# imulki/serenade

Measured on AMD Instinct MI355X. Metric: mel frames/sec converted (UNet ODE + vocoder), 80x1024, higher is better.
Workload: dtype f32

## Files before the change

### include/serenade_hip.h

```cpp
#ifndef SERENADE_HIP_H
#define SERENADE_HIP_H

#include <stdint.h>

#ifdef __cplusplus
extern "C" {
#endif

#define SRN_ABI_VERSION 4
#define SRN_MAX_TAPS 16

enum { SRN_ACT_NONE = 0, SRN_ACT_LEAKY = 1, SRN_ACT_SILU = 2, SRN_ACT_MISH = 3 };
enum { SRN_RES_NONE = 0, SRN_RES_ADD = 1, SRN_RES_AXPY = 2 };
enum {
  SRN_POST_NONE = 0,
  SRN_POST_DIV = 1,
  SRN_POST_TANH = 2,
  SRN_POST_RELU = 3,
  SRN_POST_LEAKY = 4,
  SRN_POST_GELU = 5
};
enum {
  SRN_PREC_FP32 = 0,
  SRN_PREC_BF16X3 = 1,
  SRN_PREC_BF16X6 = 2
};
enum {
  SRN_ROUTE_AUTO = 0,
  SRN_ROUTE_TILED = 1,
  SRN_ROUTE_HALO = 2,
  SRN_ROUTE_GENERIC = 3,
  SRN_ROUTE_STRIP = 4,
  SRN_ROUTE_FAST_FP32 = 5
};
enum {
  SRN_FAMILY_GENERIC = 0,
  SRN_FAMILY_F32 = 1,
  SRN_FAMILY_FAST = 2,
  SRN_FAMILY_HALO = 3,
  SRN_FAMILY_STRIP = 4
};

typedef struct SrnConvParams {
  int32_t n_batch;
  int32_t n_head;
  int32_t T_in, T_out;
  int32_t C_in;
  int32_t C_in0;
  int32_t C_w;
  int32_t N;
  int32_t N_out;
  int32_t n_taps;
  int32_t tap_off[SRN_MAX_TAPS];
  int32_t in_stride;
  int32_t pad_reflect;
  int32_t w_nmajor;
  int32_t pro_act;
  float pro_slope;
  float alpha;
  float beta;
  int32_t geglu;
  int32_t res_mode;
  int32_t post;
  float post_div;
  int32_t out_t_stride, out_t_off;
  int32_t tile;
  const float* in0; int64_t in0_bs, in0_hs; int32_t ld_in0;
  const float* in1; int64_t in1_bs; int32_t ld_in1;
  const float* w;   int64_t w_bs, w_hs; int32_t ldw;
  const float* bias;
  const int32_t* len_in;
  const int32_t* len_out;
  const float* res;  int64_t res_bs, res_hs; int32_t ld_res;
  const float* res2; int64_t res2_bs; int32_t ld_res2;
  float* out; int64_t out_bs, out_hs; int32_t ld_out;
  int32_t precision;
  int32_t route;
  void* ws; int64_t ws_bytes;
  const void* w_hi; const void* w_lo;
  float* gn_partials;
  float* out_tr; int64_t out_tr_bs; int32_t ld_out_tr; int32_t out_tr_col0;
} SrnConvParams;

int srn_abi_version(void);
const char* srn_last_error(void);

int srn_conv_gemm(const SrnConvParams* p, void* stream);
int64_t srn_conv_gemm_workspace_bytes(const SrnConvParams* p);
int srn_conv_gemm_route(const SrnConvParams* p, int32_t out[3]);

int srn_gn_mish_apply(const float* x, const float* gn_partials, const float* gamma, const float* beta,
                      const float* time_bias, int64_t time_bias_bs, const int32_t* lens, float* y, int B, int T,
                      int C, int groups, float eps, int valid_stats, void* stream);

int srn_resblock_tail(const float* c2, const float* gn_partials, const float* gamma, const float* beta,
                      const int32_t* lens, const float* r, const float* scale, const float* shift, int64_t ld_ss,
                      float* y, int B, int T, int C, int groups, float gn_eps, float ln_eps, int valid_stats,
                      void* stream);

int srn_resblock_tail_ln(const float* c2, const float* gn_partials, const float* gamma, const float* beta,
                         const int32_t* lens, const float* r, const float* scale, const float* shift, int64_t ld_ss,
                         float* y, int B, int T, int C, int groups, float gn_eps, float ln_eps, int valid_stats,
                         const float* ln2_gamma, const float* ln2_beta, float* y2, float ln2_eps, void* stream);

int srn_layernorm(const float* x, const float* gamma, const float* beta, float* y, int64_t rows, int C, float eps,
                  void* stream);

int srn_softmax_rows(float* s, const int32_t* lens, int Z, int n_head, int L, int ld, void* stream);

int srn_sinusoidal_emb(const float* t, float* out, int n, int dim, int ld, float scale, void* stream);

int srn_copy_channels(const float* src, int64_t src_bs, int ld_src, int sc0, float* dst, int64_t dst_bs, int ld_dst,
                      int dc0, int B, int T, int C, void* stream);

int srn_scatter_rows(const float* src, int64_t src_bs, int ld_src, float* dst, int64_t dst_bs, int ld_dst, int dc0,
                     const int32_t* row_off, const int32_t* n_rows, int B, int T, int C, void* stream);

int srn_transpose_ct(const float* src, float* dst, int B, int R, int Cc, int64_t src_bs, int ld_src, int64_t dst_bs,
                     int ld_dst, void* stream);
#define SRN_TR_LIST_MAX 40
typedef struct SrnTransposeList {
  int32_t n;
  int32_t pad_;
  const float* src[SRN_TR_LIST_MAX];
  float* dst[SRN_TR_LIST_MAX];
  int64_t src_bs[SRN_TR_LIST_MAX], dst_bs[SRN_TR_LIST_MAX];
  int32_t B[SRN_TR_LIST_MAX], R[SRN_TR_LIST_MAX], Cc[SRN_TR_LIST_MAX];
  int32_t ld_src[SRN_TR_LIST_MAX], ld_dst[SRN_TR_LIST_MAX];
  int32_t first_block[SRN_TR_LIST_MAX + 1];
} SrnTransposeList;
int srn_transpose_multi(const SrnTransposeList* list, void* stream);

int srn_renorm(const float* x, const float* trg_scale, const float* trg_mean, const float* voc_mean,
               const float* voc_scale, float* y, int64_t rows, int C, void* stream);

int srn_out_conv_tanh(const float* x, const float* w, const float* bias, float* y, int B, int T, int C, int k,
                      float slope, void* stream);

typedef struct SrnResUnitParams {
  int32_t n_batch, T, C;
  int32_t k, dilation;
  float slope;
  const float* x; int64_t x_bs;
  const float* w1; const float* b1; const float* w2; const float* b2;
  const void* w1_hi; const void* w2_hi;
  const float* res2; int64_t res2_bs;
  float post_div;
  float* out; int64_t out_bs;
  int32_t precision;
  int32_t route;
} SrnResUnitParams;
enum { SRN_RESUNIT_ROUTE_SHARED = 1 };

int srn_hifigan_resunit(const SrnResUnitParams* p, void* stream);

int srn_pd_gather(const float* x, const float* d, float* out, int B, int T, int C, float dilation, float slope,
                  void* stream);

int srn_gru_recur_last(const float* gi, const float* w_hh_t, const float* b_hh, float* h, int B, int T, int H,
                       void* stream);

int srn_style_token_attention_kv(const float* ref, const float* wq_t, const float* bq, const float* k, const float* v,
                                 const float* wo_t, const float* bo, float* out, int B, int Dq, int n_tok, int F,
                                 int n_head, void* stream);

int srn_pad_signal(const float* x, float* out, int B, int n, int pad, int ld, int mode, void* stream);
int srn_logmel(const float* spec, const float* mel_t, float* out, int64_t frames, int n_bins, int ld, int n_mels,
               float eps, int log_mode, void* stream);
int srn_loudness(const float* spec, const float* a_weight_db, uint32_t* gmax_ws, float* out, int B, int frames,
                 int n_bins, int ld, float amin, float top_db, float add_eps, void* stream);

int srn_rowln_fwd(const float* x, const float* m, int64_t m_bs, const float* a, int64_t a_bs, float* y, int B, int T,
                  int C, float eps, void* stream);
int srn_rowln_bwd(const float* x, const float* dy, const float* m, int64_t m_bs, float* dx, float* partial, int B, int T,
                  int C, float eps, void* stream);
int srn_rowln_chunks(int T);
int srn_gn_mish_bwd_partial(const float* h, const float* dy, const float* mean, const float* rstd, const float* gamma,
                            const float* beta, const int32_t* lens, float* partial, int B, int T, int C, int groups,
                            void* stream);
int srn_gn_mish_bwd_apply(const float* h, const float* dy, const float* mean, const float* rstd, const float* gamma,
                          const float* beta, const float* gsum, const int32_t* lens, float* dh, int B, int T, int C,
                          int groups, void* stream);
int srn_gn_chunks(int T);
int srn_gn_stats(const float* partials, float* mean, float* rstd, int B, int T, int C, int groups, float eps,
                 void* stream);
int srn_chunk_colsum(const float* partial, const float* gamma, float* col, float* gsum, int B, int n_chunk, int C,
                     int groups, void* stream);
int srn_colsum(const float* x, float* partial, float* out, int B, int64_t R, int N, int ld, void* stream);
int srn_colsum_chunks(int64_t R);
int srn_softmax_bwd(const float* p, float* dp, int64_t rows, int L, int ld, float scale, void* stream);
int srn_geglu_fwd(const float* hg, float* a, int64_t rows, int inner, void* stream);
int srn_geglu_bwd(const float* hg, const float* da, float* dhg, int64_t rows, int inner, void* stream);
int srn_adamw(float* p, const float* g, float* m, float* v, int64_t n, float lr, float beta1, float beta2, float eps,
              float weight_decay, int step, float grad_scale, void* stream);
int srn_adamw_dyn(float* p, const float* g, float* m, float* v, int64_t n, float beta1, float beta2, float eps,
                  float weight_decay, const float* dyn, void* stream);
int srn_sumsq(const float* g, int64_t n, double* partial, void* stream);
int srn_dot(const float* a, const float* b, int64_t n, double* partial, void* stream);
#define SRN_COPY_LIST_MAX 160
typedef struct SrnCopyList {
  int32_t n;
  int32_t pad_;
  const void* src[SRN_COPY_LIST_MAX];
  int64_t off[SRN_COPY_LIST_MAX];
  int64_t len[SRN_COPY_LIST_MAX];
} SrnCopyList;
int srn_multi_copy(const SrnCopyList* list, float* dst, void* stream);
int srn_sumsq_blocks(int64_t n);
int srn_weight_norm_fwd(const float* v, const float* g, float* w_packed, float* wd, float* inv_norm, int N, int C, int k,
                        void* stream);
int srn_weight_norm_bwd(const float* dw_packed, const float* v, const float* g, const float* inv_norm, float* dv,
                        float* dg, int N, int C, int k, void* stream);

typedef struct SrnWorldParams {
  int32_t n_batch, max_frames;
  int32_t fs, fft_size;
  const double* x; int64_t x_bs; const int32_t* x_len;
  const double* f0; const double* t; int64_t f_bs;
  const int32_t* n_frames;
  const double* twiddle;
  double q1, f0_floor;
  double threshold;
  double unvoiced_db;
  const double* band_window; int32_t band_window_len;
  int32_t n_bands;
  double* out0; int64_t out0_bs; int32_t ld_out0;
  double* out1; int64_t out1_bs; int32_t ld_out1;
} SrnWorldParams;
int srn_world_cheaptrick(const SrnWorldParams* p, void* stream);
int srn_world_d4c(const SrnWorldParams* p, void* stream);
int srn_world_project(const double* in, int64_t rows, int K, int ld_in, const double* mat_t, int n_out, int take_log,
                      double* out, int ld_out, void* stream);
int srn_world_pack_features(const double* a, int na, const double* b, int nb, const double* mean, const double* scale,
                            float* out, int64_t rows, int ld_out, void* stream);
int srn_wave_to_f64(const float* wave, double* out, int64_t n, int pcm16, void* stream);
int srn_f0_match_length(const double* in, int64_t in_bs, const int32_t* n_in, double* out, int64_t out_bs,
                        const int32_t* n_out, int n_batch, int max_out, void* stream);
int srn_cont_f0(const double* f0, int64_t bs, const int32_t* n_frames, double* cf0, float* uv, int32_t* ok,
                int n_batch, void* stream);
typedef struct SrnExcitationParams {
  int32_t n_batch, max_frames, fs, hop;
  const double* f0;
  const double* df_f0;
  int64_t f_bs;
  const int32_t* n_frames;
  double* phase_ws;
  const float* noise;
  float* sine;
  float sine_amp, noise_amp;
  int32_t n_df;
  float* dfs[4];
  int32_t df_upsample[4];
  double dense_factors[4];
} SrnExcitationParams;
int srn_sifigan_excitation(const SrnExcitationParams* p, void* stream);

typedef struct SrnTnGemmParams {
  int32_t n_batch, n_head;
  int32_t n_items, T_a, T_b;
  int32_t stride, n_shifts;
  int32_t shift[SRN_MAX_TAPS];
  int32_t M, N;
  const float* a; int64_t a_bs, a_hs, a_is; int32_t lda;
  const float* b; int64_t b_bs, b_hs, b_is; int32_t ldb;
  float* out; int64_t out_bs, out_hs; int32_t ldc;
  float alpha;
  float* ws; int64_t ws_bytes;
  int32_t n_inner;
  int64_t a_is2, b_is2;
  const int32_t* len_b;
  float* colsum;
  int32_t route;
} SrnTnGemmParams;
enum { SRN_TN_ROUTE_GENERAL = 1 };
int srn_tn_gemm(const SrnTnGemmParams* p, void* stream);
int64_t srn_tn_gemm_workspace_bytes(const SrnTnGemmParams* p);

int srn_bn_chunks(int64_t rows);
int srn_bn_relu_fwd(const float* x, const float* gamma, const float* beta, float* run_mean, float* run_var,
                    float* partial, float* stats, float* y, int64_t rows, int C, float eps, float momentum, void* stream);
int srn_bn_relu_bwd(const float* x, const float* y, const float* dy, const float* stats, const float* gamma,
                    float* partial, float* sums, float* dx, int64_t rows, int C, void* stream);
int srn_im2col_s2(const float* x, float* col, int B, int H, int W, int C, int ld, void* stream);
int srn_col2im_s2(const float* col, float* dx, int B, int H, int W, int C, int ld, void* stream);
int srn_gru_train_fwd(const float* gi, const float* w_hh_t, const float* b_hh, float* hs, float* gates, int B, int T,
                      int H, void* stream);
int srn_gru_train_bwd(const float* dh_last, const float* w_hh, const float* hs, const float* gates, float* dgi,
                      float* dgh, int B, int T, int H, void* stream);
int srn_token_attn_fwd(const float* q, const float* k, const float* v, float* p, float* ctx, int B, int n_tok, int F,
                       int n_head, void* stream);
int srn_token_attn_bwd(const float* dctx, const float* q, const float* k, const float* v, const float* p, float* dq,
                       float* dk_part, float* dv_part, int B, int n_tok, int F, int n_head, void* stream);

int srn_frame_stats_chunks(int T);
int srn_cvec_conv0(const float* wave, int64_t wave_bs, int n, const int32_t* lens, const float* w, float* out,
                   double* partials, int B, int T0, int C, int k, int stride, void* stream);
int srn_channel_norm_gelu(const float* x, const double* partials, int n_chunks, const int32_t* lens,
                          const float* gamma, const float* beta, float* stats, float* y, int B, int T, int C, float eps,
                          void* stream);
int srn_posconv_gelu_res(const float* x, const int32_t* lens, const float* w, const float* bias, float* y, int B,
                         int T, int C, int groups, int k, int pad, void* stream);

int srn_pad_ragged(const float* x, int64_t x_bs, const int32_t* lens, float* out, int B, int n, int pad, int ld,
                   void* stream);
int srn_mel_db(const float* spec, int ld_spec, int n_bins, const float* mel_t, const int32_t* lens, unsigned* gmax_ws,
               float* out, int ld_out, int B, int T, int n_mels, float amin, float top_db, void* stream);
int srn_trans_conv0(const float* x, int64_t x_bs, int ld_x, const int32_t* lens, const float* w, const float* bias,
                    float* out, int B, int T, int F, int C, int dilation, void* stream);
int srn_trans_pool(const float* in, const int32_t* lens, float* out, int B, int T, int F_in, int C, int C_valid,
                   int flatten, int ld_out, void* stream);
int srn_bilstm_slices(int H);
int srn_bilstm_recur(const float* g, int64_t g_bs, int ld_g, const int32_t* lens, const float* w_hh_t, float* out,
                     int64_t out_bs, int ld_out, int B, int T, int H, void* stream);

#define SRN_PYIN_MAX_FRAME 4096
#define SRN_PYIN_MAX_PERIODS 1024
#define SRN_PYIN_MAX_STATES 4096
#define SRN_PYIN_MAX_THRESHOLDS 1024
int srn_pyin_observe(const float* x, int64_t x_bs, const int32_t* lens, const int32_t* frames, const double* thresholds,
                     const double* beta_probs, const double* boltz_fact, const double* boltz_exp,
                     const double* no_trough, double* obs, double* voiced_prob, int B, int N, int T, int frame_length,
                     int win_length, int hop_length, int pad, int min_period, int max_period, int n_thresholds,
                     double sr, double fmin, double bins_per_octave, int n_bins, void* stream);
int srn_pyin_viterbi(const double* obs, const double* voiced_prob, const int32_t* frames, const double* log_band,
                     const double* log_p_init, const double* freqs, double log_tiny, double fill_na, int fill_unvoiced,
                     uint16_t* ptr_ws, int32_t* states, double* f0, uint8_t* voiced_flag, int B, int T, int n_bins,
                     int width, void* stream);

#define SRN_HARVEST_MAX_TAPS 1024
#define SRN_HARVEST_MAX_WINDOW 1536
#define SRN_HARVEST_MAX_CAND 256
#define SRN_HARVEST_MAX_RATIO 12
#define SRN_HARVEST_SMOOTH_PAD 300
int srn_harvest_decimate(const void* x, int x_is_f64, int64_t x_bs, const int32_t* lens, const double* coef, double* ws,
                         int64_t ws_stride, double* y, int64_t y_bs, int B, int N, int ratio, int lag, void* stream);
int srn_harvest_channels(const double* y, int64_t y_bs, const int32_t* ylens, const int32_t* frames, const double* taps,
                         const int32_t* tap_off, const int32_t* half_len, const double* boundary, int max_half_len,
                         double* events, int64_t ev_cap, double* raw, int B, int ch0, int n_launch, int n_ch, int F1,
                         int max_ylen, double fs, double f0_floor, double f0_ceil, void* stream);
int srn_harvest_candidates(const double* raw, const int32_t* frames, double* official, double* cand, int B, int n_ch,
                           int F1, int n_base, void* stream);
int srn_harvest_refine(const double* y, int64_t y_bs, const int32_t* ylens, const int32_t* frames, const double* cand,
                       double* refined, double* score, int B, int F1, int n_cand, double fs, double f0_floor,
                       double f0_ceil, void* stream);
int srn_harvest_contour(const double* refined, const double* score, const int32_t* frames, const int32_t* out_frames,
                        const double* smooth_coef, double* cand2, double* score2, double* fbuf, double* pool,
                        int64_t pool_stride, int32_t* sections, int sec_cap, int32_t* status, double* f0_out,
                        int64_t out_stride, int B, int F1, int n_cand, int F_out, int voice_range_minimum,
                        double frame_period, void* stream);

#ifdef __cplusplus
}
#endif
#endif
```

### serenade_amd/_lib.py

```python
import ctypes
import os
from ctypes import POINTER, c_char_p, c_double, c_float, c_int, c_int32, c_int64, c_void_p

_HERE = os.path.dirname(os.path.abspath(__file__))
LIB_PATH = os.environ.get("SERENADE_AMD_LIB") or os.path.join(_HERE, "libserenade_hip.so")

SRN_MAX_TAPS = 16
ACT_NONE, ACT_LEAKY, ACT_SILU, ACT_MISH = 0, 1, 2, 3
RES_NONE, RES_ADD, RES_AXPY = 0, 1, 2
POST_NONE, POST_DIV, POST_TANH, POST_RELU, POST_LEAKY, POST_GELU = 0, 1, 2, 3, 4, 5
PREC_FP32, PREC_BF16X3, PREC_BF16X6 = 0, 1, 2
ROUTE_AUTO, ROUTE_TILED, ROUTE_HALO, ROUTE_GENERIC, ROUTE_STRIP, ROUTE_FAST_FP32 = 0, 1, 2, 3, 4, 5
FAMILY_GENERIC, FAMILY_F32, FAMILY_FAST, FAMILY_HALO, FAMILY_STRIP = 0, 1, 2, 3, 4
RESUNIT_ROUTE_SHARED = 1
TN_ROUTE_GENERAL = 1


class SrnConvParams(ctypes.Structure):
    _fields_ = [
        ("n_batch", c_int32), ("n_head", c_int32), ("T_in", c_int32), ("T_out", c_int32),
        ("C_in", c_int32), ("C_in0", c_int32), ("C_w", c_int32), ("N", c_int32), ("N_out", c_int32),
        ("n_taps", c_int32), ("tap_off", c_int32 * SRN_MAX_TAPS), ("in_stride", c_int32),
        ("pad_reflect", c_int32), ("w_nmajor", c_int32), ("pro_act", c_int32), ("pro_slope", c_float),
        ("alpha", c_float), ("beta", c_float), ("geglu", c_int32), ("res_mode", c_int32), ("post", c_int32), ("post_div", c_float),
        ("out_t_stride", c_int32), ("out_t_off", c_int32), ("tile", c_int32),
        ("in0", c_void_p), ("in0_bs", c_int64), ("in0_hs", c_int64), ("ld_in0", c_int32),
        ("in1", c_void_p), ("in1_bs", c_int64), ("ld_in1", c_int32),
        ("w", c_void_p), ("w_bs", c_int64), ("w_hs", c_int64), ("ldw", c_int32),
        ("bias", c_void_p), ("len_in", c_void_p), ("len_out", c_void_p),
        ("res", c_void_p), ("res_bs", c_int64), ("res_hs", c_int64), ("ld_res", c_int32),
        ("res2", c_void_p), ("res2_bs", c_int64), ("ld_res2", c_int32),
        ("out", c_void_p), ("out_bs", c_int64), ("out_hs", c_int64), ("ld_out", c_int32),
        ("precision", c_int32), ("route", c_int32), ("ws", c_void_p), ("ws_bytes", c_int64),
        ("w_hi", c_void_p), ("w_lo", c_void_p), ("gn_partials", c_void_p),
        ("out_tr", c_void_p), ("out_tr_bs", c_int64), ("ld_out_tr", c_int32), ("out_tr_col0", c_int32),
    ]


class SrnResUnitParams(ctypes.Structure):
    _fields_ = [
        ("n_batch", c_int32), ("T", c_int32), ("C", c_int32), ("k", c_int32), ("dilation", c_int32),
        ("slope", c_float), ("x", c_void_p), ("x_bs", c_int64),
        ("w1", c_void_p), ("b1", c_void_p), ("w2", c_void_p), ("b2", c_void_p),
        ("w1_hi", c_void_p), ("w2_hi", c_void_p), ("res2", c_void_p), ("res2_bs", c_int64),
        ("post_div", c_float), ("out", c_void_p), ("out_bs", c_int64), ("precision", c_int32), ("route", c_int32),
    ]


SRN_COPY_LIST_MAX = 160


class SrnCopyList(ctypes.Structure):
    _fields_ = [("n", c_int32), ("pad_", c_int32), ("src", c_void_p * SRN_COPY_LIST_MAX),
                ("off", c_int64 * SRN_COPY_LIST_MAX), ("len", c_int64 * SRN_COPY_LIST_MAX)]


class SrnWorldParams(ctypes.Structure):
    _fields_ = [
        ("n_batch", c_int32), ("max_frames", c_int32), ("fs", c_int32), ("fft_size", c_int32),
        ("x", c_void_p), ("x_bs", c_int64), ("x_len", c_void_p),
        ("f0", c_void_p), ("t", c_void_p), ("f_bs", c_int64), ("n_frames", c_void_p), ("twiddle", c_void_p),
        ("q1", c_double), ("f0_floor", c_double), ("threshold", c_double), ("unvoiced_db", c_double),
        ("band_window", c_void_p), ("band_window_len", c_int32), ("n_bands", c_int32),
        ("out0", c_void_p), ("out0_bs", c_int64), ("ld_out0", c_int32),
        ("out1", c_void_p), ("out1_bs", c_int64), ("ld_out1", c_int32),
    ]


SRN_TR_LIST_MAX = 40


class SrnTransposeList(ctypes.Structure):
    _fields_ = [("n", c_int32), ("pad_", c_int32), ("src", c_void_p * SRN_TR_LIST_MAX), ("dst", c_void_p * SRN_TR_LIST_MAX),
                ("src_bs", c_int64 * SRN_TR_LIST_MAX), ("dst_bs", c_int64 * SRN_TR_LIST_MAX),
                ("B", c_int32 * SRN_TR_LIST_MAX), ("R", c_int32 * SRN_TR_LIST_MAX), ("Cc", c_int32 * SRN_TR_LIST_MAX),
                ("ld_src", c_int32 * SRN_TR_LIST_MAX), ("ld_dst", c_int32 * SRN_TR_LIST_MAX),
                ("first_block", c_int32 * (SRN_TR_LIST_MAX + 1))]


class SrnTnGemmParams(ctypes.Structure):
    _fields_ = [
        ("n_batch", c_int32), ("n_head", c_int32), ("n_items", c_int32), ("T_a", c_int32), ("T_b", c_int32),
        ("stride", c_int32), ("n_shifts", c_int32), ("shift", c_int32 * SRN_MAX_TAPS), ("M", c_int32), ("N", c_int32),
        ("a", c_void_p), ("a_bs", c_int64), ("a_hs", c_int64), ("a_is", c_int64), ("lda", c_int32),
        ("b", c_void_p), ("b_bs", c_int64), ("b_hs", c_int64), ("b_is", c_int64), ("ldb", c_int32),
        ("out", c_void_p), ("out_bs", c_int64), ("out_hs", c_int64), ("ldc", c_int32),
        ("alpha", c_float), ("ws", c_void_p), ("ws_bytes", c_int64),
        ("n_inner", c_int32), ("a_is2", c_int64), ("b_is2", c_int64), ("len_b", c_void_p), ("colsum", c_void_p),
        ("route", c_int32),
    ]


class SrnExcitationParams(ctypes.Structure):
    _fields_ = [
        ("n_batch", c_int32), ("max_frames", c_int32), ("fs", c_int32), ("hop", c_int32),
        ("f0", c_void_p), ("df_f0", c_void_p), ("f_bs", c_int64), ("n_frames", c_void_p), ("phase_ws", c_void_p),
        ("noise", c_void_p), ("sine", c_void_p), ("sine_amp", c_float), ("noise_amp", c_float), ("n_df", c_int32),
        ("dfs", c_void_p * 4), ("df_upsample", c_int32 * 4), ("dense_factors", c_double * 4),
    ]


_P = c_void_p
_SIGS = {
    "srn_abi_version": (c_int, []),
    "srn_last_error": (c_char_p, []),
    "srn_conv_gemm": (c_int, [POINTER(SrnConvParams), _P]),
    "srn_conv_gemm_workspace_bytes": (c_int64, [POINTER(SrnConvParams)]),
    "srn_conv_gemm_route": (c_int, [POINTER(SrnConvParams), POINTER(c_int32)]),
    "srn_hifigan_resunit": (c_int, [POINTER(SrnResUnitParams), _P]),
    "srn_gn_mish_apply": (c_int, [_P, _P, _P, _P, _P, c_int64, _P, _P, c_int, c_int, c_int, c_int, c_float, c_int, _P]),
    "srn_resblock_tail": (c_int, [_P, _P, _P, _P, _P, _P, _P, _P, c_int64, _P, c_int, c_int, c_int, c_int,
                                  c_float, c_float, c_int, _P]),
    "srn_resblock_tail_ln": (c_int, [_P, _P, _P, _P, _P, _P, _P, _P, c_int64, _P, c_int, c_int, c_int, c_int,
                                     c_float, c_float, c_int, _P, _P, _P, c_float, _P]),
    "srn_scatter_rows": (c_int, [_P, c_int64, c_int, _P, c_int64, c_int, c_int, _P, _P, c_int, c_int, c_int, _P]),
    "srn_layernorm": (c_int, [_P, _P, _P, _P, c_int64, c_int, c_float, _P]),
    "srn_softmax_rows": (c_int, [_P, _P, c_int, c_int, c_int, c_int, _P]),
    "srn_sinusoidal_emb": (c_int, [_P, _P, c_int, c_int, c_int, c_float, _P]),
    "srn_copy_channels": (c_int, [_P, c_int64, c_int, c_int, _P, c_int64, c_int, c_int, c_int, c_int, c_int, _P]),
    "srn_transpose_ct": (c_int, [_P, _P, c_int, c_int, c_int, c_int64, c_int, c_int64, c_int, _P]),
    "srn_transpose_multi": (c_int, [POINTER(SrnTransposeList), _P]),
    "srn_weight_norm_fwd": (c_int, [_P, _P, _P, _P, _P, c_int, c_int, c_int, _P]),
    "srn_weight_norm_bwd": (c_int, [_P, _P, _P, _P, _P, _P, c_int, c_int, c_int, _P]),
    "srn_renorm": (c_int, [_P, _P, _P, _P, _P, _P, c_int64, c_int, _P]),
    "srn_out_conv_tanh": (c_int, [_P, _P, _P, _P, c_int, c_int, c_int, c_int, c_float, _P]),
    "srn_pd_gather": (c_int, [_P, _P, _P, c_int, c_int, c_int, c_float, c_float, _P]),
    "srn_pad_signal": (c_int, [_P, _P, c_int, c_int, c_int, c_int, c_int, _P]),
    "srn_logmel": (c_int, [_P, _P, _P, c_int64, c_int, c_int, c_int, c_float, c_int, _P]),
    "srn_loudness": (c_int, [_P, _P, _P, _P, c_int, c_int, c_int, c_int, c_float, c_float, c_float, _P]),
    "srn_gru_recur_last": (c_int, [_P, _P, _P, _P, c_int, c_int, c_int, _P]),
    "srn_style_token_attention_kv": (c_int, [_P] * 8 + [c_int] * 5 + [_P]),
    "srn_rowln_fwd": (c_int, [_P, _P, c_int64, _P, c_int64, _P, c_int, c_int, c_int, c_float, _P]),
    "srn_rowln_bwd": (c_int, [_P, _P, _P, c_int64, _P, _P, c_int, c_int, c_int, c_float, _P]),
    "srn_rowln_chunks": (c_int, [c_int]),
    "srn_gn_mish_bwd_partial": (c_int, [_P] * 8 + [c_int] * 4 + [_P]),
    "srn_gn_mish_bwd_apply": (c_int, [_P] * 9 + [c_int] * 4 + [_P]),
    "srn_gn_chunks": (c_int, [c_int]),
    "srn_gn_stats": (c_int, [_P, _P, _P, c_int, c_int, c_int, c_int, c_float, _P]),
    "srn_chunk_colsum": (c_int, [_P, _P, _P, _P, c_int, c_int, c_int, c_int, _P]),
    "srn_colsum": (c_int, [_P, _P, _P, c_int, c_int64, c_int, c_int, _P]),
    "srn_colsum_chunks": (c_int, [c_int64]),
    "srn_softmax_bwd": (c_int, [_P, _P, c_int64, c_int, c_int, c_float, _P]),
    "srn_geglu_fwd": (c_int, [_P, _P, c_int64, c_int, _P]),
    "srn_geglu_bwd": (c_int, [_P, _P, _P, c_int64, c_int, _P]),
    "srn_adamw": (c_int, [_P, _P, _P, _P, c_int64, c_float, c_float, c_float, c_float, c_float, c_int, c_float, _P]),
    "srn_adamw_dyn": (c_int, [_P, _P, _P, _P, c_int64, c_float, c_float, c_float, c_float, _P, _P]),
    "srn_sumsq": (c_int, [_P, c_int64, _P, _P]),
    "srn_dot": (c_int, [_P, _P, c_int64, _P, _P]),
    "srn_multi_copy": (c_int, [POINTER(SrnCopyList), _P, _P]),
    "srn_sumsq_blocks": (c_int, [c_int64]),
    "srn_bn_chunks": (c_int, [c_int64]),
    "srn_bn_relu_fwd": (c_int, [_P] * 8 + [c_int64, c_int, c_float, c_float, _P]),
    "srn_bn_relu_bwd": (c_int, [_P] * 8 + [c_int64, c_int, _P]),
    "srn_im2col_s2": (c_int, [_P, _P] + [c_int] * 5 + [_P]),
    "srn_col2im_s2": (c_int, [_P, _P] + [c_int] * 5 + [_P]),
    "srn_gru_train_fwd": (c_int, [_P] * 5 + [c_int] * 3 + [_P]),
    "srn_gru_train_bwd": (c_int, [_P] * 6 + [c_int] * 3 + [_P]),
    "srn_token_attn_fwd": (c_int, [_P] * 5 + [c_int] * 4 + [_P]),
    "srn_token_attn_bwd": (c_int, [_P] * 8 + [c_int] * 4 + [_P]),
    "srn_tn_gemm": (c_int, [POINTER(SrnTnGemmParams), _P]),
    "srn_tn_gemm_workspace_bytes": (c_int64, [POINTER(SrnTnGemmParams)]),
    "srn_world_cheaptrick": (c_int, [POINTER(SrnWorldParams), _P]),
    "srn_world_d4c": (c_int, [POINTER(SrnWorldParams), _P]),
    "srn_world_project": (c_int, [_P, c_int64, c_int, c_int, _P, c_int, c_int, _P, c_int, _P]),
    "srn_world_pack_features": (c_int, [_P, c_int, _P, c_int, _P, _P, _P, c_int64, c_int, _P]),
    "srn_wave_to_f64": (c_int, [_P, _P, c_int64, c_int, _P]),
    "srn_f0_match_length": (c_int, [_P, c_int64, _P, _P, c_int64, _P, c_int, c_int, _P]),
    "srn_cont_f0": (c_int, [_P, c_int64, _P, _P, _P, _P, c_int, _P]),
    "srn_sifigan_excitation": (c_int, [POINTER(SrnExcitationParams), _P]),
    "srn_frame_stats_chunks": (c_int, [c_int]),
    "srn_cvec_conv0": (c_int, [_P, c_int64, c_int, _P, _P, _P, _P] + [c_int] * 5 + [_P]),
    "srn_channel_norm_gelu": (c_int, [_P, _P, c_int, _P, _P, _P, _P, _P, c_int, c_int, c_int, c_float, _P]),
    "srn_posconv_gelu_res": (c_int, [_P] * 5 + [c_int] * 6 + [_P]),
    "srn_pad_ragged": (c_int, [_P, c_int64, _P, _P, c_int, c_int, c_int, c_int, _P]),
    "srn_mel_db": (c_int, [_P, c_int, c_int, _P, _P, _P, _P, c_int, c_int, c_int, c_int, c_float, c_float, _P]),
    "srn_trans_conv0": (c_int, [_P, c_int64, c_int, _P, _P, _P, _P] + [c_int] * 5 + [_P]),
    "srn_trans_pool": (c_int, [_P, _P, _P] + [c_int] * 7 + [_P]),
    "srn_bilstm_slices": (c_int, [c_int]),
    "srn_bilstm_recur": (c_int, [_P, c_int64, c_int, _P, _P, _P, c_int64, c_int, c_int, c_int, c_int, _P]),
    "srn_pyin_observe": (c_int, [_P, c_int64] + [_P] * 9 + [c_int] * 10 + [c_double] * 3 + [c_int, _P]),
    "srn_pyin_viterbi": (c_int, [_P] * 6 + [c_double] * 2 + [c_int] + [_P] * 4 + [c_int] * 4 + [_P]),
    "srn_harvest_decimate": (c_int, [_P, c_int, c_int64, _P, _P, _P, c_int64, _P, c_int64] + [c_int] * 4 + [_P]),
    "srn_harvest_channels": (c_int, [_P, c_int64] + [_P] * 6 + [c_int, _P, c_int64, _P] + [c_int] * 6
                             + [c_double] * 3 + [_P]),
    "srn_harvest_candidates": (c_int, [_P] * 4 + [c_int] * 4 + [_P]),
    "srn_harvest_refine": (c_int, [_P, c_int64] + [_P] * 5 + [c_int] * 3 + [c_double] * 3 + [_P]),
    "srn_harvest_contour": (c_int, [_P] * 9 + [c_int64, _P, c_int, _P, _P, c_int64] + [c_int] * 5 + [c_double, _P]),
}

EXPORTS = tuple(_SIGS)

_lib = None


def lib():
    global _lib
    if _lib is None:
        if not os.path.exists(LIB_PATH):
            raise RuntimeError(
                f"{LIB_PATH} not found: build it with `python -m serenade_amd.build` "
                "(hipcc --offload-arch=gfx950). There is no CPU fallback.")
        h = ctypes.CDLL(LIB_PATH)
        for name, (res, args) in _SIGS.items():
            fn = getattr(h, name)
            fn.restype = res
            fn.argtypes = args
        if h.srn_abi_version() != 4:
            raise RuntimeError("libserenade_hip.so ABI version mismatch")
        _lib = h
    return _lib


def check(rc, what=""):
    if rc != 0:
        msg = lib().srn_last_error().decode("utf-8", "replace")
        raise RuntimeError(f"libserenade_hip {what} failed (rc={rc}): {msg}")
```

### serenade_amd/csrc/conv_f32.hip

```cpp
#include <hip/hip_runtime.h>

#include "common.h"
#include "conv_common.h"
#include "serenade_hip.h"

namespace {

constexpr int BK = 32;
constexpr int ROW = 36;
constexpr unsigned OOB = 0x80000000u;

typedef unsigned u32x4 __attribute__((ext_vector_type(4)));

struct FDiv {
  uint32_t mul, shift;
};
__device__ __forceinline__ int fdiv(const int n, const FDiv d) {
  return (int)(((uint64_t)(uint32_t)n * d.mul) >> d.shift);
}

struct F32Launch {
  int m_tiles, n_tiles, ksplit, per_slice, tiles_all;
  FDiv d_per_z, d_band, d_head, d_tiles_all, d_cpt;
};

template <int BM_, int BN_, int WM_, int WN_, int KW_, int MINW_, int PF_ = 1>
struct TCfg {
  static constexpr int BM = BM_, BN = BN_, WM = WM_, WN = WN_, KW = KW_, MINW = MINW_, PF = PF_;
  static constexpr int MT = WM / 32, NT = WN / 32;
  static constexpr int WAVES_N = BN / WN, WAVES_M = BM / WM;
  static_assert(WAVES_M * WAVES_N * KW == 4, "4 waves per workgroup");
  static constexpr int A_LD = BM / 32, B_LD = BN / 32;
  static constexpr int KK = (BK / 8) / KW;
  static_assert(KK * KW * 8 == BK, "the step divides over the wave groups");
  static constexpr int SMEM_BYTES = (BM + BN) * ROW * 4;
  static_assert((KW - 1) * WAVES_M * WAVES_N * MT * NT * 16 * 64 * 4 <= SMEM_BYTES, "join scratch fits the stage");
};

template <int MT, int NT>
__device__ __forceinline__ void f32_epilogue(const SrnConvParams& p, f32x16 (&acc)[MT][NT], const int zb, const int zh,
                                             const int t0, const int n0, const int wm0_, const int wn0_, const int lane) {
  const int wm0 = __builtin_amdgcn_readfirstlane(wm0_);
  const int wn0 = __builtin_amdgcn_readfirstlane(wn0_);
  if constexpr (NT % 2 == 0) {
    if (p.geglu) {
      conv_epilogue_impl<MT, NT, true, false>(p, acc, zb, zh, t0, n0, wm0, wn0, lane);
      return;
    }
  }
  const int li = lane & 31;
  const int lh = lane >> 5;
  int len_out = p.T_out;
  if (p.len_out) len_out = min(p.len_out[zb], p.T_out);
  const int ts = p.out_t_stride;
  const int rows_all = (p.T_out - 1) * ts + p.out_t_off;
  float* const out = p.out + (int64_t)zb * p.out_bs + (int64_t)zh * p.out_hs;
  const __amdgpu_buffer_rsrc_t rs_o =
      __builtin_amdgcn_make_buffer_rsrc(out, 0, (rows_all * p.ld_out + p.N_out) * 4, 0x00020000);
  const bool has_res = p.res_mode != SRN_RES_NONE;
  const float* const res = has_res ? p.res + (int64_t)zb * p.res_bs + (int64_t)zh * p.res_hs : out;
  const float* const res2 = p.res2 ? p.res2 + (int64_t)zb * p.res2_bs : out;
  const __amdgpu_buffer_rsrc_t rs_r = __builtin_amdgcn_make_buffer_rsrc(
      const_cast<float*>(res), 0, has_res ? (rows_all * p.ld_res + p.N_out) * 4 : 0, 0x00020000);
  const __amdgpu_buffer_rsrc_t rs_q = __builtin_amdgcn_make_buffer_rsrc(
      const_cast<float*>(res2), 0, p.res2 ? (rows_all * p.ld_res2 + p.N_out) * 4 : 0, 0x00020000);
  const bool simple = !has_res && p.res2 == nullptr && p.post == SRN_POST_NONE;
  const float alpha = p.alpha;
  const int o_v = (4 * lh * ts * p.ld_out + li) * 4;
  const int r_v = (4 * lh * ts * p.ld_res + li) * 4;
  const int q_v = (4 * lh * ts * p.ld_res2 + li) * 4;
  const int o_rs = ts * p.ld_out * 4, r_rs = ts * p.ld_res * 4, q_rs = ts * p.ld_res2 * 4;
  const int gn_mt = (p.T_out + 31) / 32, gn_nt = p.N / 32;
  const bool gn = p.gn_partials != nullptr;
  float bias_all[NT];
#pragma unroll
  for (int n = 0; n < NT; ++n) {
    const int ncol = n0 + wn0 + n * 32 + li;
    bias_all[n] = (p.bias != nullptr && ncol < p.N) ? p.bias[ncol] : 0.f;
  }

#pragma unroll
  for (int m = 0; m < MT; ++m) {
    const int tm = t0 + wm0 + m * 32;
    if (tm >= p.T_out) continue;
#pragma unroll
    for (int n = 0; n < NT; ++n) {
      const int nc0 = n0 + wn0 + n * 32;
      const bool fast = tm + 32 <= len_out && nc0 + 32 <= p.N && nc0 + 32 <= p.N_out &&
                        !(p.out_tr != nullptr && nc0 >= p.out_tr_col0);
      if (!fast) {
        f32x16(&one)[1][1] = reinterpret_cast<f32x16(&)[1][1]>(acc[m][n]);
        if (simple) conv_epilogue_impl<1, 1, false, false>(p, one, zb, zh, t0, n0, wm0 + m * 32, wn0 + n * 32, lane);
        else conv_epilogue_impl<1, 1, false, true>(p, one, zb, zh, t0, n0, wm0 + m * 32, wn0 + n * 32, lane);
        continue;
      }
      const float bias = bias_all[n];
      const int row0 = tm * ts + p.out_t_off;
      const int o_s = (row0 * p.ld_out + nc0) * 4;
      float s1 = 0.f, s2 = 0.f;
      if (simple && !gn) {
#pragma unroll
        for (int r = 0; r < 16; ++r) {
          const int dr = (r & 3) + 8 * (r >> 2);
          const float v = acc[m][n][r] * alpha + bias;
          __builtin_amdgcn_raw_buffer_store_b32(__builtin_bit_cast(unsigned, v), rs_o, o_v, o_s + dr * o_rs, 0);
        }
      } else if (simple) {
#pragma unroll
        for (int r = 0; r < 16; ++r) {
          const int dr = (r & 3) + 8 * (r >> 2);
          const float v = acc[m][n][r] * alpha + bias;
          __builtin_amdgcn_raw_buffer_store_b32(__builtin_bit_cast(unsigned, v), rs_o, o_v, o_s + dr * o_rs, 0);
          s1 += v;
          s2 += v * v;
        }
      } else {
        const int r_s = (row0 * p.ld_res + nc0) * 4, q_s = (row0 * p.ld_res2 + nc0) * 4;
        float rv[16], qv[16];
#pragma unroll
        for (int r = 0; r < 16; ++r) {
          const int dr = (r & 3) + 8 * (r >> 2);
          rv[r] = __builtin_bit_cast(float, __builtin_amdgcn_raw_buffer_load_b32(rs_r, r_v, r_s + dr * r_rs, 0));
          qv[r] = __builtin_bit_cast(float, __builtin_amdgcn_raw_buffer_load_b32(rs_q, q_v, q_s + dr * q_rs, 0));
        }
        const int res_mode = p.res_mode, post = p.post;
        const bool has_q = p.res2 != nullptr;
#pragma unroll
        for (int r = 0; r < 16; ++r) {
          const int dr = (r & 3) + 8 * (r >> 2);
          float v = acc[m][n][r] * alpha + bias;
          if (res_mode == SRN_RES_ADD) v += rv[r];
          else if (res_mode == SRN_RES_AXPY) v = rv[r] + p.beta * v;
          if (has_q) v += qv[r];
          if (post == SRN_POST_DIV) v = v / p.post_div;
          else if (post == SRN_POST_TANH) v = tanhf(v);
          else if (post == SRN_POST_RELU) v = fmaxf(v, 0.f);
          else if (post == SRN_POST_LEAKY) v = v > 0.f ? v : v * p.post_div;
          else if (post == SRN_POST_GELU) v = srn_gelu_erf(v);
          __builtin_amdgcn_raw_buffer_store_b32(__builtin_bit_cast(unsigned, v), rs_o, o_v, o_s + dr * o_rs, 0);
          s1 += v;
          s2 += v * v;
        }
      }
      if (gn) {
        s1 = wave_sum(s1);
        s2 = wave_sum(s2);
        const int gmt = tm >> 5, gnt = nc0 >> 5;
        if (lane == 0 && gmt < gn_mt && gnt < gn_nt) {
          float* gp = p.gn_partials + (((int64_t)zb * gn_mt + gmt) * gn_nt + gnt) * 2;
          gp[0] = s1;
          gp[1] = s2;
        }
      }
    }
  }
}

template <class C, int ACT>
__global__ __launch_bounds__(256, C::MINW) void conv_f32_kernel(const SrnConvParams p, const F32Launch L) {
  constexpr int BM = C::BM, BN = C::BN, MT = C::MT, NT = C::NT;
  extern __shared__ __attribute__((aligned(16))) unsigned char smem_raw[];
  float* const smem = reinterpret_cast<float*>(smem_raw);

  const int tid = threadIdx.x;
  const int lane = tid & 63;
  const int wave = __builtin_amdgcn_readfirstlane(tid >> 6);

  int logical = xcd_logical_block();
  int slice = 0;
  if (L.ksplit > 1) {
    slice = fdiv(logical, L.d_tiles_all);
    logical -= slice * L.tiles_all;
  }
  const int per_z = L.m_tiles * L.n_tiles;
  const int z = fdiv(logical, L.d_per_z);
  const int l = logical - z * per_z;
  const int band = fdiv(l, L.d_band);
  const int m0 = band * TILE_BAND;
  const int gm = min(TILE_BAND, L.m_tiles - m0);
  const int r = l - band * TILE_BAND * L.n_tiles;
  int nt_i;
  switch (gm) {
    case 8: nt_i = r >> 3; break;
    case 7: nt_i = (int)((unsigned)r / 7u); break;
    case 6: nt_i = (int)((unsigned)r / 6u); break;
    case 5: nt_i = (int)((unsigned)r / 5u); break;
    case 4: nt_i = r >> 2; break;
    case 3: nt_i = (int)((unsigned)r / 3u); break;
    case 2: nt_i = r >> 1; break;
    default: nt_i = r; break;
  }
  const int mt_i = m0 + (r - nt_i * gm);
  const int zb = fdiv(z, L.d_head);
  const int zh = z - zb * p.n_head;
  const int t0 = mt_i * BM;
  const int n0 = nt_i * BN;

  const int T_in = p.T_in;
  int len_in = T_in;
  if (p.len_in) len_in = min(p.len_in[zb], T_in);

  const int cpt = p.C_in >> 5;
  const int cp0 = p.C_in0 >> 5;
  const int steps_all = p.n_taps * cpt;
  int s_begin = 0, n_steps = steps_all;
  if (L.ksplit > 1) {
    s_begin = slice * L.per_slice;
    n_steps = max(0, min(steps_all, s_begin + L.per_slice) - s_begin);
  }

  const float* a0 = p.in0 + (int64_t)zb * p.in0_bs + (int64_t)zh * p.in0_hs;
  const float* a1 = p.in1 ? p.in1 + (int64_t)zb * p.in1_bs : a0;
  const float* wb = p.w + (int64_t)zb * p.w_bs + (int64_t)zh * p.w_hs;
  const int bytes0 = ((T_in - 1) * p.ld_in0 + p.C_in0) * 4;
  const int bytes1 = p.in1 ? ((T_in - 1) * p.ld_in1 + (p.C_in - p.C_in0)) * 4 : bytes0;
  const int bytesw = ((p.N - 1) * p.ldw + steps_all * BK) * 4;
  const __amdgpu_buffer_rsrc_t rs0 = __builtin_amdgcn_make_buffer_rsrc(const_cast<float*>(a0), 0, bytes0, 0x00020000);
  const __amdgpu_buffer_rsrc_t rs1 = __builtin_amdgcn_make_buffer_rsrc(const_cast<float*>(a1), 0, bytes1, 0x00020000);
  const __amdgpu_buffer_rsrc_t rsw = __builtin_amdgcn_make_buffer_rsrc(const_cast<float*>(wb), 0, bytesw, 0x00020000);

  const int c16 = (tid & 7) * 16;
  const int lrow = tid >> 3;
  int a_tb[C::A_LD];
#pragma unroll
  for (int i = 0; i < C::A_LD; ++i) a_tb[i] = min(t0 + lrow + 32 * i, p.T_out - 1) * p.in_stride;
  unsigned voff_b[C::B_LD];
#pragma unroll
  for (int i = 0; i < C::B_LD; ++i) voff_b[i] = __umul24((unsigned)min(n0 + lrow + 32 * i, p.N - 1), (unsigned)(p.ldw * 4)) + (unsigned)c16;
  unsigned voff_a[C::A_LD];
  int cur_tap, cur_seg, left, soff_a;
  int soff_b = s_begin * (BK * 4);
  auto a_setup = [&](const int tap, const int seg) {
    const int toff = p.tap_off[tap];
    const int ld4 = (seg == 0 ? p.ld_in0 : p.ld_in1) * 4;
#pragma unroll
    for (int i = 0; i < C::A_LD; ++i) {
      int ti = a_tb[i] + toff;
      if (p.pad_reflect) {
        const int T_ref = p.pad_reflect == 2 ? len_in : T_in;
        if (ti < 0) ti = -ti;
        if (ti >= T_ref) ti = 2 * (T_ref - 1) - ti;
      }
      voff_a[i] = (unsigned)ti < (unsigned)len_in ? __umul24((unsigned)ti, (unsigned)ld4) + (unsigned)c16 : OOB;
    }
  };
  {
    cur_tap = L.ksplit > 1 ? fdiv(s_begin, L.d_cpt) : 0;
    const int within = s_begin - cur_tap * cpt;
    cur_seg = within >= cp0 ? 1 : 0;
    const int chunk = cur_seg ? within - cp0 : within;
    a_setup(min(cur_tap, p.n_taps - 1), cur_seg);
    left = (cur_seg ? cpt - cp0 : cp0) - chunk;
    soff_a = chunk * (BK * 4);
  }

  struct Regs {
    u32x4 pa[C::A_LD];
    u32x4 pb[C::B_LD];
  };
  auto load_issue = [&](Regs& R) {
    if (cur_seg == 0) {
#pragma unroll
      for (int i = 0; i < C::A_LD; ++i) R.pa[i] = __builtin_amdgcn_raw_buffer_load_b128(rs0, voff_a[i], soff_a, 0);
    } else {
#pragma unroll
      for (int i = 0; i < C::A_LD; ++i) R.pa[i] = __builtin_amdgcn_raw_buffer_load_b128(rs1, voff_a[i], soff_a, 0);
    }
#pragma unroll
    for (int i = 0; i < C::B_LD; ++i) R.pb[i] = __builtin_amdgcn_raw_buffer_load_b128(rsw, voff_b[i], soff_b, 0);
    soff_a += BK * 4;
    soff_b += BK * 4;
  };
  auto advance = [&]() {
    if (--left == 0) {
      if (cur_seg == 0 && cp0 < cpt) {
        cur_seg = 1;
      } else {
        cur_seg = 0;
        ++cur_tap;
      }
      if (cur_tap < p.n_taps) {
        a_setup(cur_tap, cur_seg);
        left = cur_seg ? cpt - cp0 : cp0;
        soff_a = 0;
      } else {
        left = 1 << 30;
      }
    }
  };

  const float pro_slope = p.pro_slope;
  float* const st_a = smem + lrow * ROW + (tid & 7) * 4;
  float* const st_b = st_a + BM * ROW;
  auto store = [&](Regs& R) {
#pragma unroll
    for (int i = 0; i < C::A_LD; ++i) {
      float4 v = __builtin_bit_cast(float4, R.pa[i]);
      if constexpr (ACT == SRN_ACT_LEAKY) {
        v.x = fmaxf(v.x, v.x * pro_slope);
        v.y = fmaxf(v.y, v.y * pro_slope);
        v.z = fmaxf(v.z, v.z * pro_slope);
        v.w = fmaxf(v.w, v.w * pro_slope);
      }
      *reinterpret_cast<float4*>(st_a + i * 32 * ROW) = v;
    }
#pragma unroll
    for (int i = 0; i < C::B_LD; ++i) *reinterpret_cast<float4*>(st_b + i * 32 * ROW) = __builtin_bit_cast(float4, R.pb[i]);
  };

  f32x16 acc[MT][NT];
#pragma unroll
  for (int m = 0; m < MT; ++m)
#pragma unroll
    for (int n = 0; n < NT; ++n)
#pragma unroll
      for (int r16 = 0; r16 < 16; ++r16) acc[m][n][r16] = 0.f;

  const int wq = wave % (C::WAVES_M * C::WAVES_N);
  const int kg = wave / (C::WAVES_M * C::WAVES_N);
  const int wm0 = (wq / C::WAVES_N) * C::WM;
  const int wn0 = (wq % C::WAVES_N) * C::WN;
  const int li = lane & 31;
  const int lh = lane >> 5;
  const float* const fa = smem + (wm0 + li) * ROW + 4 * lh + kg * (C::KK * 8);
  const float* const fb = smem + (BM + wn0 + li) * ROW + 4 * lh + kg * (C::KK * 8);

  auto compute = [&]() {
#pragma unroll
    for (int kk = 0; kk < C::KK; ++kk) {
      float4 af[MT], bf[NT];
#pragma unroll
      for (int m = 0; m < MT; ++m) af[m] = *reinterpret_cast<const float4*>(fa + m * 32 * ROW + kk * 8);
#pragma unroll
      for (int n = 0; n < NT; ++n) bf[n] = *reinterpret_cast<const float4*>(fb + n * 32 * ROW + kk * 8);
#pragma unroll
      for (int m = 0; m < MT; ++m)
#pragma unroll
        for (int n = 0; n < NT; ++n) acc[m][n] = __builtin_amdgcn_mfma_f32_32x32x2f32(af[m].x, bf[n].x, acc[m][n], 0, 0, 0);
#pragma unroll
      for (int m = 0; m < MT; ++m)
#pragma unroll
        for (int n = 0; n < NT; ++n) acc[m][n] = __builtin_amdgcn_mfma_f32_32x32x2f32(af[m].y, bf[n].y, acc[m][n], 0, 0, 0);
#pragma unroll
      for (int m = 0; m < MT; ++m)
#pragma unroll
        for (int n = 0; n < NT; ++n) acc[m][n] = __builtin_amdgcn_mfma_f32_32x32x2f32(af[m].z, bf[n].z, acc[m][n], 0, 0, 0);
#pragma unroll
      for (int m = 0; m < MT; ++m)
#pragma unroll
        for (int n = 0; n < NT; ++n) acc[m][n] = __builtin_amdgcn_mfma_f32_32x32x2f32(af[m].w, bf[n].w, acc[m][n], 0, 0, 0);
    }
  };

  if constexpr (C::PF == 2) {
    Regs R0, R1;
    auto step = [&](Regs& R, const bool more) {
      store(R);
      __syncthreads();
      if (more) load_issue(R);
      compute();
      if (more) advance();
      __syncthreads();
    };
    if (n_steps == 1) {
      load_issue(R0);
      step(R0, false);
    } else if (n_steps > 1) {
      load_issue(R0);
      advance();
      load_issue(R1);
      advance();
      int s = 0;
      for (; s + 3 < n_steps; s += 2) {
        step(R0, true);
        step(R1, true);
      }
      if (n_steps - s == 3) {
        step(R0, true);
        step(R1, false);
        step(R0, false);
      } else {
        step(R0, false);
        step(R1, false);
      }
    }
  } else if (n_steps > 0) {
    Regs R;
    load_issue(R);
    advance();
    for (int s = 1; s < n_steps; ++s) {
      store(R);
      __syncthreads();
      load_issue(R);
      compute();
      advance();
      __syncthreads();
    }
    store(R);
    __syncthreads();
    compute();
  }

  if constexpr (C::KW > 1) {
    __syncthreads();
    float* const park = smem + wq * (MT * NT * 16 * 64) + lane;
    if (kg == 1) {
#pragma unroll
      for (int m = 0; m < MT; ++m)
#pragma unroll
        for (int n = 0; n < NT; ++n)
#pragma unroll
          for (int r16 = 0; r16 < 16; ++r16) park[((m * NT + n) * 16 + r16) * 64] = acc[m][n][r16];
    }
    __syncthreads();
    if (kg != 0) return;
#pragma unroll
    for (int m = 0; m < MT; ++m)
#pragma unroll
      for (int n = 0; n < NT; ++n)
#pragma unroll
        for (int r16 = 0; r16 < 16; ++r16) acc[m][n][r16] += park[((m * NT + n) * 16 + r16) * 64];
  }

  if (L.ksplit > 1) splitk_store<MT, NT>(p, acc, slice, z, t0, n0, wm0, wn0, lane);
  else f32_epilogue<MT, NT>(p, acc, zb, zh, t0, n0, wm0, wn0, lane);
}

FDiv make_fdiv(const uint32_t d) {
  int lg = 0;
  while ((1u << lg) < d) ++lg;
  const int k = 26 + lg;
  return FDiv{(uint32_t)(((1ull << k) + d - 1) / d), (uint32_t)k};
}

template <class C, int ACT>
int launch_f32_2(const SrnConvParams& p, hipStream_t stream, const int ksplit) {
  static SrnSmemAttr smem_attr;
  if (const int e = smem_attr.ensure(reinterpret_cast<const void*>(&conv_f32_kernel<C, ACT>), C::SMEM_BYTES)) return e;
  F32Launch L;
  L.m_tiles = (p.T_out + C::BM - 1) / C::BM;
  L.n_tiles = (p.N + C::BN - 1) / C::BN;
  L.ksplit = ksplit;
  const int cpt = p.C_in / BK;
  const int steps_all = p.n_taps * cpt;
  L.per_slice = (steps_all + ksplit - 1) / ksplit;
  const int64_t tiles_all = (int64_t)p.n_batch * p.n_head * L.m_tiles * L.n_tiles;
  const int64_t blocks = tiles_all * ksplit;
  SRN_CHECK_ARG(blocks > 0 && blocks < (1ll << 26), "conv_f32: %lld workgroups (the magic divisions hold below 2^26)",
                (long long)blocks);
  L.tiles_all = (int)tiles_all;
  L.d_per_z = make_fdiv((uint32_t)(L.m_tiles * L.n_tiles));
  L.d_band = make_fdiv((uint32_t)(TILE_BAND * L.n_tiles));
  L.d_head = make_fdiv((uint32_t)p.n_head);
  L.d_tiles_all = make_fdiv((uint32_t)tiles_all);
  L.d_cpt = make_fdiv((uint32_t)cpt);
  hipLaunchKernelGGL((conv_f32_kernel<C, ACT>), dim3((unsigned)blocks), dim3(256), C::SMEM_BYTES, stream, p, L);
  SRN_CHECK_LAUNCH();
  return 0;
}

template <class C>
int launch_f32(const SrnConvParams& p, hipStream_t stream, const int ksplit) {
  if (p.pro_act == SRN_ACT_NONE) return launch_f32_2<C, SRN_ACT_NONE>(p, stream, ksplit);
  return launch_f32_2<C, SRN_ACT_LEAKY>(p, stream, ksplit);
}

}

int srn_conv_f32_launch(const SrnConvParams& p, int tile, int ksplit, hipStream_t stream) {
  switch (tile) {
    case 5: return launch_f32<TCfg<128, 32, 32, 32, 1, 6>>(p, stream, ksplit);
    case 7: return launch_f32<TCfg<64, 64, 32, 32, 1, 6>>(p, stream, ksplit);
    case 9: return launch_f32<TCfg<64, 128, 32, 64, 1, 4>>(p, stream, ksplit);
    case 10: return launch_f32<TCfg<32, 64, 32, 32, 2, 6>>(p, stream, ksplit);
    case 11: return launch_f32<TCfg<64, 64, 32, 32, 1, 5, 2>>(p, stream, ksplit);
    default: break;
  }
  srn_set_error("conv_f32: no tile id %d", tile);
  return -1;
}
```

Before: 61250.

## Specialize f32 conv epilogue for GEGLU and direct transposed stores

```diff
diff --git a/include/serenade_hip.h b/include/serenade_hip.h
--- a/include/serenade_hip.h
+++ b/include/serenade_hip.h
@@ -31,7 +31,8 @@
   SRN_ROUTE_HALO = 2,
   SRN_ROUTE_GENERIC = 3,
   SRN_ROUTE_STRIP = 4,
-  SRN_ROUTE_FAST_FP32 = 5
+  SRN_ROUTE_FAST_FP32 = 5,
+  SRN_ROUTE_F32_BASE = 6
 };
 enum {
   SRN_FAMILY_GENERIC = 0,
diff --git a/serenade_amd/_lib.py b/serenade_amd/_lib.py
--- a/serenade_amd/_lib.py
+++ b/serenade_amd/_lib.py
@@ -11,6 +11,7 @@
 POST_NONE, POST_DIV, POST_TANH, POST_RELU, POST_LEAKY, POST_GELU = 0, 1, 2, 3, 4, 5
 PREC_FP32, PREC_BF16X3, PREC_BF16X6 = 0, 1, 2
 ROUTE_AUTO, ROUTE_TILED, ROUTE_HALO, ROUTE_GENERIC, ROUTE_STRIP, ROUTE_FAST_FP32 = 0, 1, 2, 3, 4, 5
+ROUTE_F32_BASE = 6
 FAMILY_GENERIC, FAMILY_F32, FAMILY_FAST, FAMILY_HALO, FAMILY_STRIP = 0, 1, 2, 3, 4
 RESUNIT_ROUTE_SHARED = 1
 TN_ROUTE_GENERAL = 1
diff --git a/serenade_amd/csrc/conv_f32.hip b/serenade_amd/csrc/conv_f32.hip
--- a/serenade_amd/csrc/conv_f32.hip
+++ b/serenade_amd/csrc/conv_f32.hip
@@ -37,12 +37,12 @@
   static_assert((KW - 1) * WAVES_M * WAVES_N * MT * NT * 16 * 64 * 4 <= SMEM_BYTES, "join scratch fits the stage");
 };
 
-template <int MT, int NT>
+template <int MT, int NT, bool GEGLU>
 __device__ __forceinline__ void f32_epilogue(const SrnConvParams& p, f32x16 (&acc)[MT][NT], const int zb, const int zh,
                                              const int t0, const int n0, const int wm0_, const int wn0_, const int lane) {
   const int wm0 = __builtin_amdgcn_readfirstlane(wm0_);
   const int wn0 = __builtin_amdgcn_readfirstlane(wn0_);
-  if constexpr (NT % 2 == 0) {
+  if constexpr (NT % 2 == 0 && !GEGLU) {
     if (p.geglu) {
       conv_epilogue_impl<MT, NT, true, false>(p, acc, zb, zh, t0, n0, wm0, wn0, lane);
       return;
@@ -52,6 +52,45 @@
   const int lh = lane >> 5;
   int len_out = p.T_out;
   if (p.len_out) len_out = min(p.len_out[zb], p.T_out);
+  if constexpr (GEGLU) {
+    {
+      float* const out = p.out + (int64_t)zb * p.out_bs + (int64_t)zh * p.out_hs;
+      const int ts = p.out_t_stride;
+      const int rows_all = (p.T_out - 1) * ts + p.out_t_off;
+      const __amdgpu_buffer_rsrc_t rs_o =
+          __builtin_amdgcn_make_buffer_rsrc(out, 0, (rows_all * p.ld_out + p.N_out) * 4, 0x00020000);
+      const float alpha = p.alpha;
+      const int o_v = (4 * lh * ts * p.ld_out + li) * 4;
+      const int o_rs = ts * p.ld_out * 4;
+#pragma unroll
+      for (int m = 0; m < MT; ++m) {
+        const int tm = t0 + wm0 + m * 32;
+        if (tm >= p.T_out) continue;
+#pragma unroll
+        for (int n = 0; n < NT; n += 2) {
+          const int nc0 = n0 + wn0 + n * 32;
+          const int oc0 = (nc0 >> 6) * 32;
+          if (!(tm + 32 <= len_out && nc0 + 64 <= p.N && oc0 + 32 <= p.N_out)) {
+            f32x16(&two)[1][2] = reinterpret_cast<f32x16(&)[1][2]>(acc[m][n]);
+            conv_epilogue_impl<1, 2, true, false>(p, two, zb, zh, t0, n0, wm0 + m * 32, wn0 + n * 32, lane);
+            continue;
+          }
+          const float bias_v = p.bias != nullptr ? p.bias[nc0 + li] : 0.f;
+          const float bias_g = p.bias != nullptr ? p.bias[nc0 + 32 + li] : 0.f;
+          const int o_s = ((tm * ts + p.out_t_off) * p.ld_out + oc0) * 4;
+#pragma unroll
+          for (int r = 0; r < 16; ++r) {
+            const int dr = (r & 3) + 8 * (r >> 2);
+            float v = acc[m][n][r] * alpha + bias_v;
+            const float g = acc[m][n + 1][r] * alpha + bias_g;
+            v = v * srn_gelu_erf(g);
+            __builtin_amdgcn_raw_buffer_store_b32(__builtin_bit_cast(unsigned, v), rs_o, o_v, o_s + dr * o_rs, 0);
+          }
+        }
+      }
+      return;
+    }
+  }
   const int ts = p.out_t_stride;
   const int rows_all = (p.T_out - 1) * ts + p.out_t_off;
   float* const out = p.out + (int64_t)zb * p.out_bs + (int64_t)zh * p.out_hs;
@@ -89,6 +128,24 @@
       const bool fast = tm + 32 <= len_out && nc0 + 32 <= p.N && nc0 + 32 <= p.N_out &&
                         !(p.out_tr != nullptr && nc0 >= p.out_tr_col0);
       if (!fast) {
+        if constexpr (NT == 1) {
+          if (p.out_tr != nullptr && nc0 >= p.out_tr_col0 && tm + 32 <= len_out && nc0 + 32 <= p.N &&
+              nc0 + 32 <= p.N_out && p.route != SRN_ROUTE_F32_BASE) {
+            float* const t_u = p.out_tr + (int64_t)zb * p.out_tr_bs + (int64_t)(nc0 - p.out_tr_col0) * p.ld_out_tr + tm;
+            const unsigned t_v = (unsigned)li * (unsigned)p.ld_out_tr + 4 * lh;
+            const float bias = bias_all[n];
+#pragma unroll
+            for (int gq = 0; gq < 4; ++gq) {
+              float4 v4;
+              v4.x = acc[m][n][4 * gq + 0] * alpha + bias;
+              v4.y = acc[m][n][4 * gq + 1] * alpha + bias;
+              v4.z = acc[m][n][4 * gq + 2] * alpha + bias;
+              v4.w = acc[m][n][4 * gq + 3] * alpha + bias;
+              *reinterpret_cast<float4*>(t_u + 8 * gq + t_v) = v4;
+            }
+            continue;
+          }
+        }
         f32x16(&one)[1][1] = reinterpret_cast<f32x16(&)[1][1]>(acc[m][n]);
         if (simple) conv_epilogue_impl<1, 1, false, false>(p, one, zb, zh, t0, n0, wm0 + m * 32, wn0 + n * 32, lane);
         else conv_epilogue_impl<1, 1, false, true>(p, one, zb, zh, t0, n0, wm0 + m * 32, wn0 + n * 32, lane);
@@ -156,7 +213,7 @@
   }
 }
 
-template <class C, int ACT>
+template <class C, int ACT, bool GEGLU>
 __global__ __launch_bounds__(256, C::MINW) void conv_f32_kernel(const SrnConvParams p, const F32Launch L) {
   constexpr int BM = C::BM, BN = C::BN, MT = C::MT, NT = C::NT;
   extern __shared__ __attribute__((aligned(16))) unsigned char smem_raw[];
@@ -423,7 +480,7 @@
   }
 
   if (L.ksplit > 1) splitk_store<MT, NT>(p, acc, slice, z, t0, n0, wm0, wn0, lane);
-  else f32_epilogue<MT, NT>(p, acc, zb, zh, t0, n0, wm0, wn0, lane);
+  else f32_epilogue<MT, NT, GEGLU>(p, acc, zb, zh, t0, n0, wm0, wn0, lane);
 }
 
 FDiv make_fdiv(const uint32_t d) {
@@ -433,10 +490,14 @@
   return FDiv{(uint32_t)(((1ull << k) + d - 1) / d), (uint32_t)k};
 }
 
-template <class C, int ACT>
+constexpr int GEGLU_LDS_FOUR = 40960;
+
+template <class C, int ACT, bool GEGLU>
 int launch_f32_2(const SrnConvParams& p, hipStream_t stream, const int ksplit) {
+  constexpr int kSmem = GEGLU ? GEGLU_LDS_FOUR : C::SMEM_BYTES;
+  static_assert(C::SMEM_BYTES <= kSmem, "the padded request holds the stage");
   static SrnSmemAttr smem_attr;
-  if (const int e = smem_attr.ensure(reinterpret_cast<const void*>(&conv_f32_kernel<C, ACT>), C::SMEM_BYTES)) return e;
+  if (const int e = smem_attr.ensure(reinterpret_cast<const void*>(&conv_f32_kernel<C, ACT, GEGLU>), kSmem)) return e;
   F32Launch L;
   L.m_tiles = (p.T_out + C::BM - 1) / C::BM;
   L.n_tiles = (p.N + C::BN - 1) / C::BN;
@@ -454,15 +515,21 @@
   L.d_head = make_fdiv((uint32_t)p.n_head);
   L.d_tiles_all = make_fdiv((uint32_t)tiles_all);
   L.d_cpt = make_fdiv((uint32_t)cpt);
-  hipLaunchKernelGGL((conv_f32_kernel<C, ACT>), dim3((unsigned)blocks), dim3(256), C::SMEM_BYTES, stream, p, L);
+  hipLaunchKernelGGL((conv_f32_kernel<C, ACT, GEGLU>), dim3((unsigned)blocks), dim3(256), kSmem, stream, p, L);
   SRN_CHECK_LAUNCH();
   return 0;
 }
 
 template <class C>
 int launch_f32(const SrnConvParams& p, hipStream_t stream, const int ksplit) {
-  if (p.pro_act == SRN_ACT_NONE) return launch_f32_2<C, SRN_ACT_NONE>(p, stream, ksplit);
-  return launch_f32_2<C, SRN_ACT_LEAKY>(p, stream, ksplit);
+  if constexpr (C::NT % 2 == 0) {
+    if (p.geglu && p.route != SRN_ROUTE_F32_BASE) {
+      if (p.pro_act == SRN_ACT_NONE) return launch_f32_2<C, SRN_ACT_NONE, true>(p, stream, ksplit);
+      return launch_f32_2<C, SRN_ACT_LEAKY, true>(p, stream, ksplit);
+    }
+  }
+  if (p.pro_act == SRN_ACT_NONE) return launch_f32_2<C, SRN_ACT_NONE, false>(p, stream, ksplit);
+  return launch_f32_2<C, SRN_ACT_LEAKY, false>(p, stream, ksplit);
 }
 
 }
```

Measured after the change: 61600 (median of 6 runs). Within noise of the previous version (+0.6%).
